# finsberg/fenicsx-beat

Hardware: AMD Instinct MI355X
Metric: node_updates_per_sec (higher is better)
Workload: dtype f64

## Files before the change

### fenicsx-beat_amd/csrc/beat_pde.hip

```cpp
#include "beat_pde_internal.h"

#include <algorithm>
#include <cmath>
#include <cstdlib>
#include <cstring>
#include <vector>

const int beat_pde_detail::kOffsets[45] = {0, 0, 0,  1, 0, 0,  -1, 0, 0,  0, 1, 0,  0, -1, 0,  0, 0, 1,  0, 0, -1,
                          1, 1, 0,  -1, -1, 0,  0, 1, 1,  0, -1, -1,  1, 0, 1,  -1, 0, -1,
                          1, 1, 1,  -1, -1, -1};

namespace {
using namespace beat_pde_detail;

template <int TX_, int TY_>
struct Tile {
  static constexpr int TX = TX_, TY = TY_;
  static constexpr int PITCH = TX + 2;
  static constexpr int SLOT = (TY + 2) * PITCH;
  static constexpr int NLOAD = (SLOT + BEAT_BLOCK - 1) / BEAT_BLOCK;
  static constexpr int ROWS_PER_THREAD = TY / (BEAT_BLOCK / TX);
  static_assert(TX * TY == 1024 && ROWS_PER_THREAD == 4, "tile must hold 1024 nodes");
};
constexpr int TARGET_BLOCKS = 1024;
// ... 243 lines not shown
  }
}

__device__ __forceinline__ void beat_pcg_roll(double* st) {
  st[BETA] = st[RZN] / st[RZ];
  st[RZ] = st[RZN];
  st[RR] = st[RRN];
  st[ITERS] += 1.0;
  const double tr = st[RTOL] * st[RTOL] * st[BB];
  if (st[RR] <= st[TOL2]) {
    st[STOP] = 1.0;
    st[REASON] = st[RR] <= tr ? 2.0 : 3.0;
  } else if (st[ITERS] >= st[MAXIT]) {
    st[STOP] = 1.0;
    st[REASON] = -3.0;
  }
}
__device__ __forceinline__ void beat_pcg_begin(double* st, double rtol, double atol, double max_it) {
  const double bb = st[BB], rr = st[RR];
  const double tr = rtol * rtol * bb, ta = atol * atol;
  const double tol2 = tr > ta ? tr : ta;
  st[TOL2] = tol2;
  st[ITERS] = 0.0;
  st[NUPD] = 0.0;
  st[RTOL] = rtol;
  st[ATOL] = atol;
  st[MAXIT] = max_it;
  st[BETA] = 0.0;
  st[RR0] = rr;
  const bool done = rr <= tol2;
  st[STOP] = done ? 1.0 : 0.0;
  st[REASON] = done ? (rr <= tr ? 2.0 : 3.0) : 0.0;
}
__global__ __launch_bounds__(BEAT_BLOCK) void reduce_partials_kernel(const double* __restrict__ partials, int count, int nsum, double* out,
                                                                     const double* st, double* counter, int then, double* roll_st,
                                                                     double rtol, double atol, double max_it) {
  __shared__ double red[4];
  if (st != nullptr && st[STOP] != 0.0) return;
  if (counter != nullptr && threadIdx.x == 0) counter[0] += 1.0;
  for (int k = 0; k < nsum; ++k) {
    double s = 0.0;
    for (int i = threadIdx.x; i < count; i += BEAT_BLOCK) s += partials[(int64_t)k * BEAT_MAX_PARTIALS + i];
    s = beat_block_sum(s, red);
    if (threadIdx.x == 0) out[k] = s;
  }
  if (then != 0 && threadIdx.x == 0) {
    if (then == 1) beat_pcg_roll(roll_st);
    else beat_pcg_begin(roll_st, rtol, atol, max_it);
  }
}

__global__ void pcg_begin_kernel(double* st, double rtol, double atol, double max_it) { beat_pcg_begin(st, rtol, atol, max_it); }

__global__ void pcg_next_kernel(double* st) {
  if (st[STOP] != 0.0) return;
  beat_pcg_roll(st);
}

template <bool VAR>
__global__ __launch_bounds__(BEAT_BLOCK) void cg_update_kernel(Geom g, const double* __restrict__ st,
                                                               double* __restrict__ x,
                                                               double* __restrict__ r,
                                                               const double* __restrict__ p,
                                                               const double* __restrict__ q,
                                                               const double* __restrict__ dinv,
                                                               double dinv_i, double* __restrict__ partials) {
  __shared__ double red[4];
  if (st[STOP] != 0.0) return;
  const double alpha = st[RZ] / st[PQ];
  const int lane = threadIdx.x & 63, wave = threadIdx.x >> 6;
  const int nrows = g.ny * g.nz;
  double s_rz = 0.0, s_rr = 0.0;
  for (int row = blockIdx.x * 4 + wave; row < nrows; row += gridDim.x * 4) {
    const int iz = row / g.ny, iy = row - iz * g.ny;
    const int tyz = 3 * axis_type(iy, g.ny, 1, 1) + 9 * axis_type(iz, g.nz, g.z_lo_phys, g.z_hi_phys);
    const int64_t base = (int64_t)row * g.nx;
    for (int ix = lane; ix < g.nx; ix += 64) {
      const int type = axis_type(ix, g.nx, 1, 1) + tyz;
      const int64_t i = base + ix;
      const double di = VAR ? dinv[i] : (type == 13) ? dinv_i : dinv[type];
      const double pi = p[i], qi = q[i];
      const double xi = fma(alpha, pi, x[i]);
// ... 184 lines not shown
  g.ny = (int)n[1];
  g.nz = (int)n[2];
  g.plane = n[0] * n[1];
  g.z_lo_phys = z_lo_phys ? 1 : 0;
  g.z_hi_phys = z_hi_phys ? 1 : 0;
  int tile_tx = g.nx >= 256 ? 256 : g.nx >= 128 ? 128 : 64;
  if (const char* e = std::getenv("BEAT_TILE_TX")) {
    const int v = std::atoi(e);
    if (v == 64 || v == 128 || v == 256) tile_tx = v;
  }
  g.tile_tx = tile_tx;
  const int TX = tile_tx, TY = 1024 / tile_tx;
  g.tiles_x = (g.nx + TX - 1) / TX;
  g.tiles_y = (g.ny + TY - 1) / TY;
  const int tiles = g.tiles_x * g.tiles_y;
  int nchunks = std::max(1, (TARGET_BLOCKS + tiles - 1) / tiles);
  nchunks = std::min(nchunks, g.nz);
  g.zc = (g.nz + nchunks - 1) / nchunks;
  g.nchunks = (g.nz + g.zc - 1) / g.zc;
  const int64_t total = (int64_t)tiles * g.nchunks;
  if (total > BEAT_MAX_PARTIALS) {
    g.nchunks = std::max(1, (int)(BEAT_MAX_PARTIALS / tiles));
    g.zc = (g.nz + g.nchunks - 1) / g.nchunks;
    g.nchunks = (g.nz + g.zc - 1) / g.zc;
  }
  BEAT_REQUIRE((int64_t)tiles * g.nchunks <= BEAT_MAX_PARTIALS, "xy plane too large: %d tiles", tiles);
  g.total = tiles * g.nchunks;
  g.z_lo = 0;
  g.z_hi = g.nz;
  g.part_off = 0;
  p->n = n[0] * n[1] * n[2];
  const int64_t rows = (int64_t)g.ny * g.nz;
  p->vec_grid = (unsigned)std::min<int64_t>(2048, std::max<int64_t>(1, (rows + 3) / 4));
  std::memcpy(p->h_mass, host_mass_tab, sizeof(p->h_mass));
  std::memcpy(p->h_stiff, host_stiff_tab, sizeof(p->h_stiff));
  BEAT_HIP_CHECK(hipSetDevice(ctx->device));
  BEAT_HIP_CHECK(hipMalloc(&p->d_tabs, sizeof(double) * (4 * 27 * TABW + 32)));
  BEAT_HIP_CHECK(hipMalloc(&p->d_st, sizeof(double) * BEAT_ST_DOUBLES));
  BEAT_HIP_CHECK(hipMalloc(&p->d_alphas, sizeof(double) * PRING_MAX));
  BEAT_HIP_CHECK(hipMemsetAsync(p->d_st, 0, sizeof(double) * BEAT_ST_DOUBLES, ctx->stream));
  const int rc = upload_tables(p);
  if (rc) return rc;
  *out = p;
  return BEAT_OK;
}


extern "C" int beat_pde_set_ghost_types(beat_pde* pde, int ghost_lo_type, int ghost_hi_type) {
  BEAT_REQUIRE(pde != nullptr, "null pde");
  BEAT_REQUIRE(ghost_lo_type >= 0 && ghost_lo_type <= 2 && ghost_hi_type >= 0 && ghost_hi_type <= 2, "node types are 0, 1 or 2");
  pde->ghost_lo_tz = ghost_lo_type;
  pde->ghost_hi_tz = ghost_hi_type;
  return BEAT_OK;
}

extern "C" int beat_pde_destroy(beat_pde* pde) {
  if (pde == nullptr) return BEAT_OK;
  if (pde->open.on && pde->ctx != nullptr) (void)hipStreamSynchronize(pde->ctx->stream);
  (void)hipFree(pde->d_tabs);
  (void)hipFree(pde->d_st);
  (void)hipFree(pde->d_alphas);
  (void)hipFree(pde->d_batch_st);
  (void)hipFree(pde->d_hist_alloc);
  if (pde->h_st) (void)hipHostFree(pde->h_st);
  if (pde->ev_st) (void)hipEventDestroy(pde->ev_st);
  (void)hipFree(pde->v_A);
// ... 65 lines not shown
}

template <int MODE>
static void launch_stencil(const beat_pde* pde, const StencilArgs& a, const Geom* range = nullptr) {
  const Geom& g = range ? *range : pde->g;
  if (g.total <= 0) return;
  const dim3 grid(stencil_grid(g)), block(BEAT_BLOCK);
  hipStream_t s = pde->ctx->stream;
  switch (g.tile_tx) {
    case 256: BEAT_KERNEL((stencil_kernel<MODE, Tile<256, 4>>), grid, block, 0, s, g, a); break;
    case 128: BEAT_KERNEL((stencil_kernel<MODE, Tile<128, 8>>), grid, block, 0, s, g, a); break;
    default: BEAT_KERNEL((stencil_kernel<MODE, Tile<64, 16>>), grid, block, 0, s, g, a); break;
  }
}

extern "C" int beat_pde_apply(beat_pde* pde, int which, const double* dev_x, double* dev_y) {
  BEAT_REQUIRE(pde != nullptr && dev_x && dev_y, "null argument");
  BEAT_REQUIRE(which >= 0 && which < 4, "which must be 0..3");
  BEAT_REQUIRE(which >= 2 || pde->have_dt, "beat_pde_set_timestep has not been called");
  BEAT_REQUIRE(dev_x != dev_y, "in-place apply is not supported");
  if (pde->var) return beat_var_apply(pde, which, dev_x, dev_y);
  const double* host_tab = which == 0 ? pde->h_A : which == 1 ? pde->h_B : which == 2 ? pde->h_mass : pde->h_stiff;
  StencilArgs a{};
  a.x = dev_x;
  a.y = dev_y;
  a.tab = pde->d_tab(which);
  a.ci = interior(host_tab);
  launch_stencil<MODE_APPLY>(pde, a);
  BEAT_LAUNCH_CHECK();
  return BEAT_OK;
}

int beat_pde_launch_reduce(beat_pde* pde, int count, int nsum, double* out, const double* st, double* counter, int then, double* roll_st,
                           double rtol, double atol, int max_it) {
  static const bool fuse = [] {
    const char* e = std::getenv("BEAT_PCG_FUSE");
    return !(e && e[0] == '0');
  }();
  BEAT_KERNEL(reduce_partials_kernel, dim3(1), dim3(BEAT_BLOCK), 0, pde->ctx->stream, (const double*)pde->ctx->d_partials, count, nsum, out, st,
              counter, fuse ? then : 0, roll_st, rtol, atol, (double)max_it);
  BEAT_LAUNCH_CHECK();
  if (then != 0 && !fuse) {
    if (then == 1) BEAT_KERNEL(pcg_next_kernel, dim3(1), dim3(1), 0, pde->ctx->stream, roll_st);
    else BEAT_KERNEL(pcg_begin_kernel, dim3(1), dim3(1), 0, pde->ctx->stream, roll_st, rtol, atol, (double)max_it);
    BEAT_LAUNCH_CHECK();
  }
  return BEAT_OK;
}

extern "C" int beat_pde_rhs(beat_pde* pde, const double* dev_v_prev, const double* const* host_dev_stim_w,
                            const double* host_stim_amp, int n_stim, double* dev_x, double* dev_r,
                            double* dev_p, double* dev_red) {
  BEAT_REQUIRE(pde != nullptr && dev_v_prev && dev_x && dev_r && dev_p && dev_red, "null argument");
  BEAT_REQUIRE(pde->have_dt, "beat_pde_set_timestep has not been called");
  BEAT_REQUIRE(n_stim >= 0 && n_stim <= BEAT_MAX_STIM, "at most %d stimuli", BEAT_MAX_STIM);
  BEAT_REQUIRE(dev_r != dev_v_prev && dev_p != dev_v_prev && dev_r != dev_p, "r, p must be distinct work fields");
  BEAT_REQUIRE(!pde->guess_pending, "the previous solve's deferred update has not been applied");
  beat_guess_skip(pde);
  if (pde->var)
    return beat_var_rhs(pde, dev_v_prev, host_dev_stim_w, host_stim_amp, n_stim, dev_x, dev_r, dev_p, dev_red);
  StencilArgs a{};
  a.x = dev_v_prev;
  a.y = dev_r;
  a.y2 = dev_p;
  a.y3 = (dev_x == dev_v_prev) ? nullptr : dev_x;
  a.tab = pde->d_tab(2);
  a.tab2 = pde->d_tab(3);
  a.dinv = pde->d_dinv();
  a.ci = interior(pde->h_mass);
  a.ci2 = interior(pde->h_stiff);
  a.dinv_i = pde->h_dinv[13];
  a.cm = pde->C_m;
  a.omt_dt = (1.0 - pde->theta) * pde->dt;
  a.dt = pde->dt;
  a.nstim = 0;
  for (int k = 0; k < n_stim; ++k) {
// ... 401 lines not shown
  }
  beat_guess_advance(pde);
  return due;
}

extern "C" int beat_pde_solve(beat_pde* pde, const double* dev_v_prev,
                              const double* const* host_dev_stim_w, const double* host_stim_amp,
                              int n_stim, double* dev_x, double* dev_work, double rtol, double atol,
                              int max_it, beat_ksp_info* info) {
  return beat_pde_solve_ex(pde, dev_v_prev, host_dev_stim_w, host_stim_amp, n_stim, dev_x, dev_work, rtol, atol, max_it,
                           0, info, nullptr);
}

bool beat_solve_lazy_available(const beat_pde* pde) {
  return pde != nullptr && pde->g.z_lo_phys && pde->g.z_hi_phys && !beat_small_available(pde) && pde->pc_ncoef == 1 &&
         (beat_rr_available(pde) || pde->var);
}

static int solve_enqueue_iterations(beat_pde* pde, int count) {
  beat_pde::OpenSolve& o = pde->open;
  const int64_t fld = beat_pde_field_stride(pde);
  double* r = o.work + pde->g.plane;
  double* q = r + fld;
  double* ring = q + 2 * fld;
  double* st = pde->d_st;
  const int PR = pde->ring;
  int rc;
  for (int it = 0; it < count; ++it) {
    const int i = o.launched + it, slot = i % PR;
    double* p_cur = ring + (int64_t)slot * fld;
    const double* p_old = ring + (int64_t)((i + PR - 1) % PR) * fld;
    if (o.kind == 0) {
      double* rbuf[2] = {r, q};
      if ((rc = beat_rr_pdot(pde, st, rbuf[i & 1], p_old, p_cur))) return rc;
      if ((rc = beat_rr_rupd(pde, st, rbuf[i & 1], rbuf[(i + 1) & 1], p_cur, slot))) return rc;
      if (slot == PR - 1) {
        if ((rc = beat_pde_x_flush_terms(pde, st, o.x, ring, fld, i + 1 - PR, 1, beat_guess_terms(pde, i + 1 - PR)))) return rc;
      }
    } else {
      double* p_next = ring + (int64_t)((i + 1) % PR) * fld;
      if (o.pdot) {
        if ((rc = beat_vtl_pdot(pde, st, r, p_old, p_cur, q, i == 0))) return rc;
      } else if ((rc = beat_pde_spmv_dot(pde, p_cur, q, st))) {
        return rc;
      }
      if ((rc = o.pdot ? beat_var_update_r(pde, st, r, q, slot, true) : beat_pde_cg_update_r(pde, st, r, q, slot))) return rc;
      if (slot == PR - 1) {
        if ((rc = beat_pde_x_flush_terms(pde, st, o.x, ring, fld, i + 1 - PR, 1, beat_guess_terms(pde, i + 1 - PR)))) return rc;
      }
      if (!o.pdot && (rc = beat_pde_cg_next_oop(pde, st, r, p_cur, p_next))) return rc;
    }
  }
  o.launched += count;
  return BEAT_OK;
}

int beat_solve_begin(beat_pde* pde, const double* dev_v_prev, const double* const* host_dev_stim_w, const double* host_stim_amp, int n_stim,
                     double* dev_x, double* dev_work, double rtol, double atol, int max_it) {
  BEAT_REQUIRE(pde != nullptr && dev_work != nullptr && dev_v_prev && dev_x, "null argument");
  BEAT_REQUIRE(beat_solve_lazy_available(pde), "this operator's solves are not of the kind that can be left open");
  BEAT_REQUIRE(!pde->open.on, "the previous solve has not been finished (beat_pde_solve_end)");
  BEAT_REQUIRE(max_it >= 0, "max_it must be >= 0");
  BEAT_REQUIRE(pde->have_dt, "beat_pde_set_timestep has not been called");
  BEAT_REQUIRE(n_stim >= 0 && n_stim <= BEAT_MAX_STIM, "at most %d stimuli", BEAT_MAX_STIM);
  BEAT_REQUIRE(!pde->guess_pending, "the previous solve's deferred update has not been applied");
  beat_ctx* ctx = pde->ctx;
  if (pde->h_st == nullptr) {
// ... 213 lines not shown
```

### fenicsx-beat_amd/csrc/beat_pde_internal.h

```cpp
#pragma once
#include "beat_common.h"

#include <algorithm>
#include <cstdlib>
#include <vector>

namespace beat_pde_detail {

enum St { BB = 0, RZ, RR, PQ, RZN, RRN, TOL2, BETA, STOP, ITERS, REASON, RTOL, ATOL, MAXIT, NUPD, RR0, ALPHA };
constexpr int BEAT_ST_DOUBLES = 32;
constexpr int PRING = 6;
constexpr int PRING_MAX = 12;
constexpr int TABW = 16;

extern const int kOffsets[45];

struct Geom {
  int nx, ny, nz;
  int64_t plane;
  int tiles_x, tiles_y, nchunks, zc, total;
  int z_lo_phys, z_hi_phys;
  int tile_tx;
  int z_lo, z_hi;
  int part_off;
};

enum { MODE_APPLY = 0, MODE_SPMV_DOT = 1, MODE_RHS = 2, MODE_PC = 3 };

}

struct beat_pde {
  beat_ctx* ctx = nullptr;
  beat_pde_detail::Geom g{};
  int64_t n = 0;
  double h_mass[27 * 15], h_stiff[27 * 15];
  double h_A[27 * 15], h_B[27 * 15], h_dinv[27];
  bool have_dt = false;
  double C_m = 1.0, theta = 0.5, dt = 0.0;
  double* d_tabs = nullptr;
  double* d_st = nullptr;
  int last_iters = -1;
  int z_last_iters = -1;
  unsigned vec_grid = 1;
  double* d_alphas = nullptr;
  struct OpenSolve {
    bool on = false;
    int kind = 0;
    bool pdot = false;
    const double* v_prev = nullptr;
    double* x = nullptr;
    double* work = nullptr;
    double rtol = 0.0, atol = 0.0;
    int max_it = 0, launched = 0;
    void* comm = nullptr;
    bool rr = false, merged = false, vpdot = false;
    int limit = 0;
  } open;
  struct FuseBegin {
    bool on = false, done = false;
    double rtol = 0.0, atol = 0.0;
    int max_it = 0;
  } fuse_begin;
  double* h_st = nullptr;
  hipEvent_t ev_st = nullptr;
  beat_ksp_info last_info{};
  bool applied_behind = false;
  beat_pde_detail::GuessTerms applied_terms{};
  int last_rc = 0;
  int ring = beat_pde_detail::PRING;
  int last_base = 0;
  double* d_batch_st = nullptr;
  int ghost_lo_tz = 1, ghost_hi_tz = 1;
  int single_reduction = -1;
  int guess_order = 0;
  int auto_cur = 3;
  int auto_next = 3;
  int auto_e_order = 0;
  double auto_score[4] = {0.0, 0.0, 0.0, 0.0};
  int auto_seen[4] = {0, 0, 0, 0};
  int auto_since_probe = 0, auto_probe_up = 1;
  double* d_hist[3] = {nullptr, nullptr, nullptr};
  double* d_guess = nullptr;
  double* d_hist_alloc = nullptr;
  int hist_fields = 0;
  int hist_n = 0;
  beat_pde_detail::GuessTerms guess{};
  bool guess_pending = false;
  beat_pde_detail::GuessTerms guess_final{};
  int rhs_part_blocks = 0;
  void* vrr = nullptr;
  int vrr_part_blocks = 0;
  void* vtl = nullptr;
  bool small_enabled = true;
  int pc_ncoef = 1;
  double pc_coef[8] = {1.0};
  bool var = false;
  const double* v_mass = nullptr;
  const double* v_stiff = nullptr;
  double* v_A = nullptr;
  double* v_dinv = nullptr;
  double* v_B = nullptr;
  double* v_gc0 = nullptr;
  bool v_gc0_valid = false;
  bool v_pdot_dist = false;
  int64_t v_ld = 0;
  int* v_seg = nullptr;
  std::vector<int> h_seg;
  unsigned long long* v_segmask = nullptr;
  int* v_seg_tiled = nullptr;
  unsigned long long* v_segmask_tiled = nullptr;
  const double* d_tab(int which) const { return d_tabs + (size_t)which * 27 * beat_pde_detail::TABW; }
  const double* d_dinv() const { return d_tabs + (size_t)4 * 27 * beat_pde_detail::TABW; }
  const double* dinv_arg() const { return var ? v_dinv : d_dinv(); }
};

inline int beat_pde_first_chunk(const beat_pde* pde) {
  static const int extra = [] {
    const char* e = std::getenv("BEAT_CHUNK_EXTRA");
    return e ? std::max(0, std::atoi(e)) : 1;
  }();
  return pde->last_iters >= 0 ? std::max(1, pde->last_iters + extra) : 8;
}

int beat_pde_launch_reduce(beat_pde* pde, int count, int nsum, double* out, const double* st, double* counter = nullptr, int then = 0,
                           double* roll_st = nullptr, double rtol = 0.0, double atol = 0.0, int max_it = 0);

int beat_var_form_A(beat_pde* pde);
int beat_var_apply(beat_pde* pde, int which, const double* dev_x, double* dev_y);
int beat_var_rhs(beat_pde* pde, const double* dev_v_prev, const double* const* host_dev_stim_w,
                 const double* host_stim_amp, int n_stim, double* dev_x, double* dev_r, double* dev_p, double* dev_red,
                 const double* dev_e = nullptr,
                 int part = -1);
int beat_var_spmv_dot(beat_pde* pde, const double* dev_p, double* dev_q, double* dev_st);
int beat_var_spmv_dot_part(beat_pde* pde, const double* dev_p, double* dev_q, double* dev_st, int part);
int beat_var_update_r(beat_pde* pde, double* dev_st, double* dev_r, const double* dev_q, int slot, bool roll = false);
int beat_var_pupdate_oop(beat_pde* pde, double* dev_st, const double* dev_r, const double* dev_p_cur, double* dev_p_next);
int beat_var_flush(beat_pde* pde, const double* dev_st, double* dev_x, const double* dev_ring0, int64_t field_stride,
                   int ring_base, int only_if_full, const beat_pde_detail::GuessTerms& gt);

void beat_guess_begin(beat_pde* pde);
void beat_guess_skip(beat_pde* pde);
beat_pde_detail::GuessTerms beat_guess_terms(const beat_pde* pde, int ring_base);
bool beat_guess_end(beat_pde* pde, int nupd, bool deferred);
int beat_pde_x_flush_terms(beat_pde* pde, const double* dev_st, double* dev_x, const double* dev_ring0, int64_t field_stride,
                           int ring_base, int only_if_full, const beat_pde_detail::GuessTerms& gt);

void beat_guess_advance(beat_pde* pde);
void beat_guess_observe(beat_pde* pde, int iterations);
int beat_guess_policy(beat_pde* pde);

int beat_vrr_setup(beat_pde* pde, const std::vector<unsigned long long>& host_tissue_flags);
void beat_vrr_destroy(beat_pde* pde);
bool beat_vrr_available(const beat_pde* pde);
int beat_vrr_spmv_dot(beat_pde* pde, const double* dev_p, double* dev_q, double* dev_st, int part);

int beat_vtl_setup(beat_pde* pde, const std::vector<unsigned long long>& host_tissue_flags);
void beat_vtl_destroy(beat_pde* pde);
bool beat_vtl_available(const beat_pde* pde);
int beat_vtl_spmv_dot(beat_pde* pde, const double* dev_p, double* dev_q, double* dev_st);
bool beat_vtl_parts_available(const beat_pde* pde);
bool beat_vtl_pdot_dist_available(const beat_pde* pde);
int beat_vtl_pdot_part(beat_pde* pde, double* dev_st, const double* dev_r, const double* dev_p_old, double* dev_p_new, double* dev_q,
                       int first, int part);
int beat_vtl_spmv_dot_part(beat_pde* pde, const double* dev_p, double* dev_q, double* dev_st, int part);
bool beat_vtl_pdot_available(const beat_pde* pde);
bool beat_vtl_rhs_available(const beat_pde* pde);
bool beat_vtl_rhs_wanted(const beat_pde* pde);
int beat_vtl_rhs(beat_pde* pde, const double* dev_v_prev, const double* const* host_dev_stim_w, const double* host_stim_amp, int n_stim,
                 double* dev_x, double* dev_r, double* dev_p, double* dev_t, double* dev_red, const double* dev_e);
int beat_vtl_pdot(beat_pde* pde, double* dev_st, const double* dev_r, const double* dev_p_old, double* dev_p_new, double* dev_q, int first);

bool beat_solve_lazy_available(const beat_pde* pde);
struct beat_comm;
int beat_dist_solve_begin(beat_pde* pde, beat_comm* comm, const double* dev_v_prev, const double* const* host_dev_stim_w,
                          const double* host_stim_amp, int n_stim, double* dev_x, double* dev_work, double rtol, double atol, int max_it);
int beat_dist_solve_end(beat_pde* pde, int defer_flush, beat_ksp_info* info, int* host_pending, bool* needed_more);
int beat_solve_begin(beat_pde* pde, const double* dev_v_prev, const double* const* host_dev_stim_w, const double* host_stim_amp, int n_stim,
                     double* dev_x, double* dev_work, double rtol, double atol, int max_it);
int beat_solve_end(beat_pde* pde, int defer_flush, beat_ksp_info* info, int* host_pending, bool* needed_more);

bool beat_small_available(const beat_pde* pde);
int beat_small_launch(beat_pde* pde, const double* dev_v_prev, const double* const* host_dev_stim_w,
                      const double* host_stim_amp, int n_stim, double* dev_x, double rtol, double atol, int max_it,
                      double* dev_st);
int beat_small_solve(beat_pde* pde, const double* dev_v_prev, const double* const* host_dev_stim_w,
                     const double* host_stim_amp, int n_stim, double* dev_x, double rtol, double atol, int max_it,
                     beat_ksp_info* info);

bool beat_rr_available(const beat_pde* pde);
int beat_rr_rhs(beat_pde* pde, const double* dev_v_prev, const double* const* host_dev_stim_w, const double* host_stim_amp,
                int n_stim, double* dev_x, double* dev_r, double* dev_st, int part = -1);
int beat_rr_pdot(beat_pde* pde, double* dev_st, const double* dev_r, const double* dev_p_old, double* dev_p_new);
int beat_rr_pdot_part(beat_pde* pde, double* dev_st, const double* dev_r, const double* dev_p_old, double* dev_p_new,
                      int part);
int beat_rr_rupd(beat_pde* pde, double* dev_st, const double* dev_r, double* dev_r_new, const double* dev_p, int slot,
                 bool roll = true);
int beat_rr_next(beat_pde* pde, double* dev_st);
int beat_rr_udot_part(beat_pde* pde, double* dev_st, const double* dev_r, int part);
int beat_rr_merged_next(beat_pde* pde, double* dev_st, int slot);
int beat_rr_prupd(beat_pde* pde, double* dev_st, const double* dev_r, const double* dev_p_old, double* dev_p_new,
                  double* dev_r_new);
```

### fenicsx-beat_amd/csrc/beat_pde_rr.hip

```cpp
#include "beat_pde_internal.h"

#include <algorithm>
#include <cmath>
#include <cstddef>
#include <cstdlib>

namespace {
using namespace beat_pde_detail;

constexpr int SEG = 62;

struct Coef {
  double c[15];
};

struct RGeom {
  int nx, ny, nz;
  int64_t plane;
  int ry;
  int nsegx, nrb, nchunks, zc;
  int total_waves, total_blocks;
  int z_lo_phys, z_hi_phys;
  int z_lo, z_hi;
  int part_off;
// ... 75 lines not shown
  const int hi = __builtin_amdgcn_update_dpp(__builtin_amdgcn_readlane(__double2hiint(h), src_lane), __double2hiint(v), 0x138, 0xf, 0xf, false);
  return __hiloint2double(hi, lo);
}
__device__ __forceinline__ double from_right_h(double v, double h, int src_lane) {
  const int lo = __builtin_amdgcn_update_dpp(__builtin_amdgcn_readlane(__double2loint(h), src_lane), __double2loint(v), 0x130, 0xf, 0xf, false);
  const int hi = __builtin_amdgcn_update_dpp(__builtin_amdgcn_readlane(__double2hiint(h), src_lane), __double2hiint(v), 0x130, 0xf, 0xf, false);
  return __hiloint2double(hi, lo);
}
#ifndef BEAT_RR_ALIGN_RHS
#define BEAT_RR_ALIGN_RHS 0
#endif
constexpr bool rr_aligned_mode(int mode) {
  return BEAT_RR_ALIGN == 1 && BEAT_RR_BUF != 0 && (mode == 0 || mode == 1 || mode == 3 || mode == 4 || (mode == 2 && BEAT_RR_ALIGN_RHS == 1));
}

__device__ __forceinline__ int axis_type3(int i, int n, int lo_phys, int hi_phys) {
  if (n == 1 && lo_phys && hi_phys) return 1;
  if (i == 0 && lo_phys) return 0;
  if (i == n - 1 && hi_phys) return 2;
  return 1;
}

__device__ __forceinline__ int xcd_block(int b, int total) {
  const int per = (total + 7) >> 3;
  return (b & 7) * per + (b >> 3);
}

#ifndef BEAT_RR_WAVES_RHS
#define BEAT_RR_WAVES_RHS 3
#endif
#ifndef BEAT_RR_WAVES_IT
#define BEAT_RR_WAVES_IT 1
#endif
template <int MODE, int RY, int PD, bool GUESS = false>
__global__ __launch_bounds__(BEAT_BLOCK, (GUESS && RY == 2 && PD == 1) ? BEAT_RR_WAVES_RHS : ((MODE == RR_PDOT || MODE == RR_RUPD) && PD == 1 ? BEAT_RR_WAVES_IT : 1)) void rr_kernel(RGeom g, RArgs a, const double* __restrict__ X,
                                                        const double* __restrict__ X2, double* __restrict__ Y,
                                                        double* __restrict__ Y2) {
  constexpr int NR = RY + 2;
  constexpr int NE = GUESS ? NR : 1;
  constexpr bool FORM = MODE == RR_PDOT || MODE == RR_UDOT || MODE == RR_PRUPD;
  constexpr bool OLD = MODE == RR_PDOT || MODE == RR_PRUPD;
  constexpr bool RAW = MODE == RR_UDOT || MODE == RR_PRUPD;
  constexpr int NW = RAW ? RY : 1;
  constexpr bool BUF = BEAT_RR_BUF == 1 || (BEAT_RR_BUF == 2 && (MODE != RR_RHS || BEAT_RR_ALIGN_RHS == 1));
  constexpr bool ALIGNED = rr_aligned_mode(MODE);
  static_assert(!ALIGNED || BUF, "aligned segments come with the raw-buffer loads");
  constexpr int SEGW = ALIGNED ? 64 : SEG;
  static_assert(!GUESS || MODE == RR_RHS, "the initial guess enters the right-hand side only");
  __shared__ double red[4];
  __shared__ double s_dinv[32];
  __shared__ double s_tab[27 * TABW];
  __shared__ double s_tab2[MODE == RR_RHS ? 27 * TABW : 1];
  __shared__ double s_taba[GUESS ? 27 * TABW : 1];
  if (MODE != RR_RHS) {
    if (a.st[STOP] != 0.0) return;
  }
  for (int i = threadIdx.x; i < 27 * TABW; i += BEAT_BLOCK) {
    s_tab[i] = a.tab[i];
    if (MODE == RR_RHS) s_tab2[i] = a.tab2[i];
    if (GUESS) s_taba[i] = a.taba[i];
  }
  if (threadIdx.x < 27) s_dinv[threadIdx.x] = a.dinv[threadIdx.x];
  __syncthreads();
  const int lane = threadIdx.x & 63;
  const int blk = xcd_block(blockIdx.x, g.total_blocks);
  const int w = blk * 4 + (threadIdx.x >> 6);
  int seg = w % g.nsegx;
  int rb = (w / g.nsegx) % g.nrb;
  int chunk = w / (g.nsegx * g.nrb);
  bool wave_ok = blk < g.total_blocks && w < g.total_waves;
  if (g.nrg > 0) {
    seg = blk % g.nsegx;
    rb = ((blk / g.nsegx) % g.nrg) * 4 + (int)(threadIdx.x >> 6);
    chunk = blk / (g.nsegx * g.nrg);
    wave_ok = blk < g.total_blocks && rb < g.nrb;
  }
  const int gx = seg * SEGW + (ALIGNED ? 0 : -1) + lane;
  const int y0 = rb * RY - 1;
  const int zb = g.z_lo + chunk * g.zc;
  const int ze = wave_ok ? min(zb + g.zc, g.z_hi) : zb;
  const bool x_in = wave_ok && gx >= 0 && gx < g.nx;
  const bool x_out = x_in && (ALIGNED || (lane >= 1 && lane <= SEG));
  const int tx = axis_type3(gx, g.nx, 1, 1);
  bool row_in[NR];
  int txy[NR];
  int off[NR];
  const int cx = min(max(gx, 0), g.nx - 1);
#pragma unroll
  for (int r = 0; r < NR; ++r) {
// ... 53 lines not shown
  for (int zz = zb - 2 - PD; zz < ze; zz += PD) {
#pragma unroll
  for (int u = 0; u < PD; ++u) {
    const int z = zz + u;
    if (z < ze) {
    const int k = z + 1;
    if (k >= zb - 1 && k <= ze) {
      [[maybe_unused]] const bool zok = (k >= 0 || !g.z_lo_phys) && (k < g.nz || !g.z_hi_phys);
      const int tz9 = 9 * (k < 0 ? g.ghost_lo_tz : k >= g.nz ? g.ghost_hi_tz : axis_type3(k, g.nz, g.z_lo_phys, g.z_hi_phys));
      const bool own_plane = (k >= zb && k < ze) || (k == -1 && zb == 0 && !g.z_lo_phys) ||
                             (k == g.nz && ze == g.nz && !g.z_hi_phys);
#pragma unroll
      for (int r = 0; r < NR; ++r) {
        double c = ra[u][r];
        if (RAW && r >= 1 && r <= RY) Rwp[RAW ? r - 1 : 0] = c;
        if (FORM) {
          const int type = txy[r] + tz9;
          const double di = s_dinv[type];
          c = have_old ? fma(beta, rb2[u][r], di * ra[u][r]) : di * ra[u][r];
        }
        if constexpr (!BUF) c = (zok && row_in[r]) ? c : 0.0;
        Cp[r] = c;
        if (GUESS) {
          constexpr int q = GUESS ? 1 : 0;
          if constexpr (BUF)
            Ep[r * q] = c + re1[u][r * q];
          else
            Ep[r * q] = (zok && row_in[r]) ? c + re1[u][r * q] : 0.0;
        }
        if (OLD) {
          if (own_plane && r >= 1 && r <= RY && x_out && row_in[r])
            rr_store(&Y[(int64_t)k * g.plane + (int64_t)(y0 + r) * g.nx + gx], c);
        }
      }
      if constexpr (ALIGNED) {
        double hc = rha[u];
        if (FORM) {
          const double di = s_dinv[htxy + tz9];
          hc = have_old ? fma(beta, rhb[u], di * rha[u]) : di * rha[u];
        }
        Hp = hc;
        if (GUESS) HEp = hc + rhb[u];
      }
    }
    double rv[RY];
    if (MODE == RR_RUPD) {
#pragma unroll
      for (int j = 0; j < RY; ++j) rv[j] = rvn[u][j];
      if (z + PD >= zb && z + PD < ze) {
        const double* __restrict__ br = X2 + (int64_t)(z + PD) * g.plane;
#pragma unroll
        for (int j = 0; j < RY; ++j) rvn[u][j] = BUF ? rr_buf_load(br, pbytes, (unsigned)off[j + 1]) : br[off[j + 1]];
      }
    }
    {
      const int kf = k + PD;
      if (kf >= zb - 1 && kf <= ze) {
        const int cz = min(max(kf, -1), g.nz);
        const double* __restrict__ bx = X + (int64_t)cz * g.plane;
        const double* __restrict__ bx2 = (OLD && have_old) ? X2 + (int64_t)cz * g.plane : bx;
        if constexpr (BUF) {
          const unsigned pb = ((kf >= 0 || !g.z_lo_phys) && (kf < g.nz || !g.z_hi_phys)) ? pbytes : 0u;
#pragma unroll
          for (int r = 0; r < NR; ++r) {
            ra[u][r] = rr_buf_load(bx, pb, (unsigned)off[r]);
            if (OLD) rb2[u][r] = rr_buf_load(bx2, pb, (unsigned)off[r]);
// ... 113 lines not shown
            ev[8] = eL0[rm];
            ev[9] = Ep[rp];
            ev[10] = Em[rm];
            ev[11] = eRp[re_];
            ev[12] = eLm[re_];
            ev[13] = eRp[rp];
            ev[14] = eLm[rm];
            double se = 0.0;
            if (type != 13) {
#pragma unroll
              for (int k = 0; k < 15; ++k) se = fma(s_taba[type * TABW + k], ev[k], se);
            } else {
#pragma unroll
              for (int k = 0; k < 15; ++k) se = fma(az.cia.c[k], ev[k], se);
            }
            rr -= se;
          }
          const double zz = di * rr;
          rr_store(&Y[gi], rr);
          if (Y2 != nullptr) Y2[gi] = v[0];
          acc0 = fma(b, b, acc0);
          acc1 = fma(rr, zz, acc1);
          acc2 = fma(rr, rr, acc2);
        } else {
          double di = s_dinv[13];
          if (type != 13) {
            s = 0.0;
#pragma unroll
            for (int k = 0; k < 15; ++k) s = fma(s_tab[type * TABW + k], v[k], s);
            di = s_dinv[type];
          }
          if (MODE == RR_PDOT) {
            acc0 = fma(v[0], s, acc0);
          } else if (MODE == RR_UDOT) {
            const double ri = Rw0[RAW ? j : 0];
            acc0 = fma(v[0], s, acc0);
            acc1 = fma(ri, v[0], acc1);
            acc2 = fma(ri, ri, acc2);
          } else if (MODE == RR_PRUPD) {
            rr_store(&Y2[gi], fma(-alpha, s, Rw0[RAW ? j : 0]));
          } else {
            const double ri = fma(-alpha, s, rv[j]);
            rr_store(&Y[gi], ri);
            acc0 = fma(ri * di, ri, acc0);
            acc1 = fma(ri, ri, acc1);
          }
        }
      }
    }
    }
#pragma unroll
    for (int r = 0; r < NR; ++r) {
      Cm[r] = C0[r];
      C0[r] = Cp[r];
    }
    if constexpr (ALIGNED) {
      Hm = H0;
      H0 = Hp;
      if (GUESS) {
        HEm = HE0;
        HE0 = HEp;
      }
    }
    if (GUESS) {
#pragma unroll
      for (int r = 0; r < NE; ++r) {
        Em[r] = E0[r];
        E0[r] = Ep[r];
      }
    }
    if (RAW) {
#pragma unroll
      for (int j = 0; j < NW; ++j) Rw0[j] = Rwp[j];
    }
    }
  }
  }

  if (MODE == RR_PDOT) {
    const double s0 = beat_block_sum(acc0, red);
    if (threadIdx.x == 0) a.partials[g.part_off + blockIdx.x] = s0;
  } else if (MODE == RR_RUPD) {
    const double s0 = beat_block_sum(acc0, red);
    const double s1 = beat_block_sum(acc1, red);
    if (threadIdx.x == 0) {
      a.partials[g.part_off + blockIdx.x] = s0;
      a.partials[BEAT_MAX_PARTIALS + g.part_off + blockIdx.x] = s1;
    }
  } else if (MODE == RR_PRUPD) {
  } else {
    const double s0 = beat_block_sum(acc0, red);
    const double s1 = beat_block_sum(acc1, red);
    const double s2 = beat_block_sum(acc2, red);
    if (threadIdx.x == 0) {
      a.partials[g.part_off + blockIdx.x] = s0;
      a.partials[BEAT_MAX_PARTIALS + g.part_off + blockIdx.x] = s1;
      a.partials[2 * BEAT_MAX_PARTIALS + g.part_off + blockIdx.x] = s2;
    }
  }
}

__global__ void rr_next_kernel(double* st) {
  if (st[STOP] != 0.0) return;
  st[BETA] = st[RZN] / st[RZ];
  st[RZ] = st[RZN];
  st[RR] = st[RRN];
  st[ITERS] += 1.0;
  const double tr = st[RTOL] * st[RTOL] * st[BB];
  if (st[RR] <= st[TOL2]) {
    st[STOP] = 1.0;
    st[REASON] = st[RR] <= tr ? 2.0 : 3.0;
  } else if (st[ITERS] >= st[MAXIT]) {
// ... 80 lines not shown
  g.nsegx = (f.nx + segw - 1) / segw;
  g.nrb = (f.ny + RY - 1) / RY;
  const int nzr = std::max(0, z_hi - z_lo);
  g.nrg = (mode >= 0 && ((rr_by_rows_mask() >> mode) & 1)) ? (g.nrb + 3) / 4 : 0;
  const int64_t per_layer = g.nrg > 0 ? (int64_t)g.nsegx * g.nrg : ((int64_t)g.nsegx * g.nrb + 3) / 4;
  const int target = rr_target_blocks(nodes);
  int nchunks = (int)std::max<int64_t>(1, (target + per_layer - 1) / per_layer);
  nchunks = std::max(1, std::min(nchunks, nzr));
  g.zc = std::max(1, (nzr + nchunks - 1) / nchunks);
  g.nchunks = (nzr + g.zc - 1) / g.zc;
  while ((int64_t)g.nsegx * g.nrb * g.nchunks > (int64_t)2 * BEAT_MAX_PARTIALS && g.nchunks > 1) {
    g.zc *= 2;
    g.nchunks = (nzr + g.zc - 1) / g.zc;
  }
  g.total_waves = g.nsegx * g.nrb * g.nchunks;
  g.total_blocks = (g.total_waves + 3) / 4;
  if (g.nrg > 0) {
    g.total_blocks = g.nsegx * g.nrg * g.nchunks;
    g.total_waves = g.total_blocks * 4;
  }
  return g;
}

RGeom make_geom(const beat_pde* pde) { return make_geom(pde, 0, pde->g.nz, 0); }

inline int grid_blocks(const RGeom& g) { return ((g.total_blocks + 7) / 8) * 8; }

Coef interior_row(const double* tab) {
  Coef c;
  for (int k = 0; k < 15; ++k) c.c[k] = tab[13 * 15 + k];
  return c;
}

template <int MODE, bool GUESS = false>
void launch_rr(const beat_pde* pde, const RGeom& g, const RArgs& a) {
  if (g.total_blocks <= 0) return;
  const dim3 grid((unsigned)grid_blocks(g)), block(BEAT_BLOCK);
  hipStream_t s = pde->ctx->stream;
#define BEAT_RR_LAUNCH(RYV, PDV) \
  BEAT_KERNEL((rr_kernel<MODE, RYV, PDV, GUESS>), grid, block, 0, s, g, a, a.x, GUESS ? a.e : a.x2, a.y, a.y2)
  const int pd = rr_prefetch();
  if (g.ry == 2) {
    if (pd == 2) BEAT_RR_LAUNCH(2, 2); else if (pd == 3) BEAT_RR_LAUNCH(2, 3); else BEAT_RR_LAUNCH(2, 1);
  } else {
    if (pd == 2) BEAT_RR_LAUNCH(4, 2); else if (pd == 3) BEAT_RR_LAUNCH(4, 3); else BEAT_RR_LAUNCH(4, 1);
  }
#undef BEAT_RR_LAUNCH
}
}

bool beat_rr_available(const beat_pde* pde) {
  if (pde->var || pde->pc_ncoef != 1) return false;
  if (const char* e = std::getenv("BEAT_RR")) {
    if (e[0] == '0') return false;
  }
  const RGeom g = make_geom(pde);
  const RGeom gb = make_geom(pde, 0, 1, 0);
  return (int64_t)grid_blocks(g) + 2 * grid_blocks(gb) <= BEAT_MAX_PARTIALS;
}

int beat_rr_rhs(beat_pde* pde, const double* dev_v_prev, const double* const* host_dev_stim_w, const double* host_stim_amp,
                int n_stim, double* dev_x, double* dev_r, double* dev_st, int part) {
  const GuessTerms& gt = pde->guess;
  const bool guess = gt.d != nullptr && gt.use_e;
  static const int guess_rows = [] {
    const char* e = std::getenv("BEAT_RR_GUESS_RY");
    const int v = e ? std::atoi(e) : 2;
    return v == 4 ? 4 : 2;
  }();
  const int rows = guess ? guess_rows : 0;
  RArgs a{};
  a.x = dev_v_prev;
  a.y = dev_r;
// ... 26 lines not shown
  auto launch = [&](const RGeom& g) {
    if (guess)
      launch_rr<RR_RHS, true>(pde, g, a);
    else
      launch_rr<RR_RHS>(pde, g, a);
    return g.total_blocks > 0 ? grid_blocks(g) : 0;
  };
  const Geom& f = pde->g;
  if (part < 0) {
    const int nb = launch(make_geom(pde, 0, f.nz, 0, rows, RR_RHS));
    BEAT_LAUNCH_CHECK();
    if (pde->fuse_begin.on) {
      pde->fuse_begin.done = true;
      return beat_pde_launch_reduce(pde, nb, 3, dev_st, nullptr, nullptr, 2, dev_st, pde->fuse_begin.rtol, pde->fuse_begin.atol,
                                    pde->fuse_begin.max_it);
    }
    return beat_pde_launch_reduce(pde, nb, 3, dev_st, nullptr);
  }
  const int lo = f.z_lo_phys ? 0 : 1, hi = f.nz - (f.z_hi_phys ? 0 : 1);
  const RGeom gi = make_geom(pde, lo, std::max(lo, hi), 0, rows, RR_RHS);
  if (part == 0) {
    launch(gi);
    BEAT_LAUNCH_CHECK();
    return BEAT_OK;
  }
  int off = gi.total_blocks > 0 ? grid_blocks(gi) : 0;
  if (!f.z_lo_phys) off += launch(make_geom(pde, 0, 1, off, rows, RR_RHS));
  if (!f.z_hi_phys && (f.nz > 1 || f.z_lo_phys)) off += launch(make_geom(pde, f.nz - 1, f.nz, off, rows, RR_RHS));
  BEAT_LAUNCH_CHECK();
  BEAT_REQUIRE(off <= BEAT_MAX_PARTIALS, "too many block partials");
  return beat_pde_launch_reduce(pde, off, 3, dev_st, nullptr);
}

int beat_rr_pdot_part(beat_pde* pde, double* dev_st, const double* dev_r, const double* dev_p_old, double* dev_p_new,
                      int part) {
  const Geom& f = pde->g;
  RArgs a{};
  a.x = dev_r;
  a.x2 = dev_p_old;
  a.y = dev_p_new;
  a.tab = pde->d_tab(0);
  a.dinv = pde->d_dinv();
  a.ci = interior_row(pde->h_A);
  a.dinv_i = pde->h_dinv[13];
  a.partials = pde->ctx->d_partials;
  a.st = dev_st;
  const int lo = f.z_lo_phys ? 0 : 1, hi = f.nz - (f.z_hi_phys ? 0 : 1);
  const RGeom gi = make_geom(pde, lo, std::max(lo, hi), 0, 0, RR_PDOT);
  if (part == 0) {
    launch_rr<RR_PDOT>(pde, gi, a);
    BEAT_LAUNCH_CHECK();
    return BEAT_OK;
  }
  int off = gi.total_blocks > 0 ? grid_blocks(gi) : 0;
  if (!f.z_lo_phys) {
    const RGeom gb = make_geom(pde, 0, 1, off, 0, RR_PDOT);
    launch_rr<RR_PDOT>(pde, gb, a);
    off += grid_blocks(gb);
  }
  if (!f.z_hi_phys && (f.nz > 1 || f.z_lo_phys)) {
    const RGeom gb = make_geom(pde, f.nz - 1, f.nz, off, 0, RR_PDOT);
    launch_rr<RR_PDOT>(pde, gb, a);
    off += grid_blocks(gb);
  }
  BEAT_LAUNCH_CHECK();
  BEAT_REQUIRE(off <= BEAT_MAX_PARTIALS, "too many block partials");
  return beat_pde_launch_reduce(pde, off, 1, dev_st + PQ, dev_st);
}

int beat_rr_pdot(beat_pde* pde, double* dev_st, const double* dev_r, const double* dev_p_old, double* dev_p_new) {
  if (int rc = beat_rr_pdot_part(pde, dev_st, dev_r, dev_p_old, dev_p_new, 0)) return rc;
  return beat_rr_pdot_part(pde, dev_st, dev_r, dev_p_old, dev_p_new, 1);
}

int beat_rr_rupd(beat_pde* pde, double* dev_st, const double* dev_r, double* dev_r_new, const double* dev_p, int slot,
                 bool roll) {
  const RGeom g = make_geom(pde, 0, pde->g.nz, 0, 0, RR_RUPD);
  RArgs a{};
  a.x = dev_p;
  a.x2 = dev_r;
  a.y = dev_r_new;
  a.tab = pde->d_tab(0);
  a.dinv = pde->d_dinv();
  a.ci = interior_row(pde->h_A);
  a.dinv_i = pde->h_dinv[13];
  a.partials = pde->ctx->d_partials;
  a.st = dev_st;
  a.alphas = pde->d_alphas;
  a.slot = slot;
  launch_rr<RR_RUPD>(pde, g, a);
  BEAT_LAUNCH_CHECK();
  return beat_pde_launch_reduce(pde, grid_blocks(g), 2, dev_st + RZN, dev_st, dev_st + NUPD, roll ? 1 : 0, dev_st);
}

int beat_rr_udot_part(beat_pde* pde, double* dev_st, const double* dev_r, int part) {
  static_assert(RZN == PQ + 1 && RRN == PQ + 2, "the three sums travel as one all-reduce of dev_st[PQ..RRN]");
  const Geom& f = pde->g;
  RArgs a{};
  a.x = dev_r;
  a.x2 = dev_r;
  a.tab = pde->d_tab(0);
  a.dinv = pde->d_dinv();
  a.ci = interior_row(pde->h_A);
  a.dinv_i = pde->h_dinv[13];
  a.partials = pde->ctx->d_partials;
// ... 55 lines not shown
```

Measured before the change: 10.79 billion.

## Predict CG convergence in the p-dot pass to skip the final residual update

The p-dot kernel now also accumulates r·q and q·q next to p·q, and the reduction kernel gains a predict mode. Using these three sums it computes the next residual norm by recurrence, with a floating-point error bound derived from the reduction depth. When that prediction safely decides convergence, it writes alpha and stops the solve, so the separate residual-update pass and its reduction are skipped on the last iteration. The cost is extra shared-memory traffic and two more dot products in every p-dot pass. It only runs when both z boundaries are physical and is on by default.

```diff
diff --git a/fenicsx-beat_amd/csrc/beat_pde.hip b/fenicsx-beat_amd/csrc/beat_pde.hip
--- a/fenicsx-beat_amd/csrc/beat_pde.hip
+++ b/fenicsx-beat_amd/csrc/beat_pde.hip
@@ -299,9 +299,30 @@
   st[STOP] = done ? 1.0 : 0.0;
   st[REASON] = done ? (rr <= tr ? 2.0 : 3.0) : 0.0;
 }
+__device__ __forceinline__ void beat_pcg_predict(double* st, double* alpha_slot, double c) {
+  st[PQ] = st[PQS];
+  const double alpha = st[RZ] / st[PQ];
+  const double rr = st[RR], rq = st[RQ], qq = st[QQ];
+  const double rho = fma(alpha, fma(alpha, qq, -2.0 * rq), rr);
+  const double m = sqrt(rr) + fabs(alpha) * sqrt(qq);
+  const double e = c * m * m;
+  const double tr = st[RTOL] * st[RTOL] * st[BB];
+  if (!(rho + e <= st[TOL2]) || !(e <= 0x1p-20 * rho)) return;
+  double reason;
+  if (rho + e <= tr) reason = 2.0;
+  else if (rho - e > tr) reason = 3.0;
+  else return;
+  *alpha_slot = alpha;
+  st[RR] = rho > 0.0 ? rho : 0.0;
+  st[ITERS] += 1.0;
+  st[NUPD] += 1.0;
+  st[REASON] = reason;
+  st[STOP] = 1.0;
+}
 __global__ __launch_bounds__(BEAT_BLOCK) void reduce_partials_kernel(const double* __restrict__ partials, int count, int nsum, double* out,
                                                                      const double* st, double* counter, int then, double* roll_st,
-                                                                     double rtol, double atol, double max_it) {
+                                                                     double rtol, double atol, double max_it, double* alpha_slot,
+                                                                     double bound_c) {
   __shared__ double red[4];
   if (st != nullptr && st[STOP] != 0.0) return;
   if (counter != nullptr && threadIdx.x == 0) counter[0] += 1.0;
@@ -313,8 +334,14 @@
   }
   if (then != 0 && threadIdx.x == 0) {
     if (then == 1) beat_pcg_roll(roll_st);
+    else if (then == 3) beat_pcg_predict(roll_st, alpha_slot, bound_c);
     else beat_pcg_begin(roll_st, rtol, atol, max_it);
   }
+}
+
+__global__ void pcg_predict_kernel(double* st, double* alpha_slot, double c) {
+  if (st[STOP] != 0.0) return;
+  beat_pcg_predict(st, alpha_slot, c);
 }
 
 __global__ void pcg_begin_kernel(double* st, double rtol, double atol, double max_it) { beat_pcg_begin(st, rtol, atol, max_it); }
@@ -565,6 +592,7 @@
   p->n = n[0] * n[1] * n[2];
   const int64_t rows = (int64_t)g.ny * g.nz;
   p->vec_grid = (unsigned)std::min<int64_t>(2048, std::max<int64_t>(1, (rows + 3) / 4));
+  if (const char* e = std::getenv("BEAT_PCG_PREDICT_STOP")) p->predict_stop = e[0] != '0';
   std::memcpy(p->h_mass, host_mass_tab, sizeof(p->h_mass));
   std::memcpy(p->h_stiff, host_stiff_tab, sizeof(p->h_stiff));
   BEAT_HIP_CHECK(hipSetDevice(ctx->device));
@@ -696,16 +724,17 @@
 }
 
 int beat_pde_launch_reduce(beat_pde* pde, int count, int nsum, double* out, const double* st, double* counter, int then, double* roll_st,
-                           double rtol, double atol, int max_it) {
+                           double rtol, double atol, int max_it, double* alpha_slot, double bound_c) {
   static const bool fuse = [] {
     const char* e = std::getenv("BEAT_PCG_FUSE");
     return !(e && e[0] == '0');
   }();
   BEAT_KERNEL(reduce_partials_kernel, dim3(1), dim3(BEAT_BLOCK), 0, pde->ctx->stream, (const double*)pde->ctx->d_partials, count, nsum, out, st,
-              counter, fuse ? then : 0, roll_st, rtol, atol, (double)max_it);
+              counter, fuse ? then : 0, roll_st, rtol, atol, (double)max_it, alpha_slot, bound_c);
   BEAT_LAUNCH_CHECK();
   if (then != 0 && !fuse) {
     if (then == 1) BEAT_KERNEL(pcg_next_kernel, dim3(1), dim3(1), 0, pde->ctx->stream, roll_st);
+    else if (then == 3) BEAT_KERNEL(pcg_predict_kernel, dim3(1), dim3(1), 0, pde->ctx->stream, roll_st, alpha_slot, bound_c);
     else BEAT_KERNEL(pcg_begin_kernel, dim3(1), dim3(1), 0, pde->ctx->stream, roll_st, rtol, atol, (double)max_it);
     BEAT_LAUNCH_CHECK();
   }
@@ -1173,7 +1202,7 @@
     const double* p_old = ring + (int64_t)((i + PR - 1) % PR) * fld;
     if (o.kind == 0) {
       double* rbuf[2] = {r, q};
-      if ((rc = beat_rr_pdot(pde, st, rbuf[i & 1], p_old, p_cur))) return rc;
+      if ((rc = beat_rr_pdot(pde, st, rbuf[i & 1], p_old, p_cur, slot))) return rc;
       if ((rc = beat_rr_rupd(pde, st, rbuf[i & 1], rbuf[(i + 1) & 1], p_cur, slot))) return rc;
       if (slot == PR - 1) {
         if ((rc = beat_pde_x_flush_terms(pde, st, o.x, ring, fld, i + 1 - PR, 1, beat_guess_terms(pde, i + 1 - PR)))) return rc;
diff --git a/fenicsx-beat_amd/csrc/beat_pde_internal.h b/fenicsx-beat_amd/csrc/beat_pde_internal.h
--- a/fenicsx-beat_amd/csrc/beat_pde_internal.h
+++ b/fenicsx-beat_amd/csrc/beat_pde_internal.h
@@ -7,7 +7,7 @@
 
 namespace beat_pde_detail {
 
-enum St { BB = 0, RZ, RR, PQ, RZN, RRN, TOL2, BETA, STOP, ITERS, REASON, RTOL, ATOL, MAXIT, NUPD, RR0, ALPHA };
+enum St { BB = 0, RZ, RR, PQ, RZN, RRN, TOL2, BETA, STOP, ITERS, REASON, RTOL, ATOL, MAXIT, NUPD, RR0, ALPHA, PQS, RQ, QQ };
 constexpr int BEAT_ST_DOUBLES = 32;
 constexpr int PRING = 6;
 constexpr int PRING_MAX = 12;
@@ -69,6 +69,8 @@
   int last_rc = 0;
   int ring = beat_pde_detail::PRING;
   int last_base = 0;
+  bool predict_stop = true;
+  double predict_c = 0.0;
   double* d_batch_st = nullptr;
   int ghost_lo_tz = 1, ghost_hi_tz = 1;
   int single_reduction = -1;
@@ -123,7 +125,8 @@
 }
 
 int beat_pde_launch_reduce(beat_pde* pde, int count, int nsum, double* out, const double* st, double* counter = nullptr, int then = 0,
-                           double* roll_st = nullptr, double rtol = 0.0, double atol = 0.0, int max_it = 0);
+                           double* roll_st = nullptr, double rtol = 0.0, double atol = 0.0, int max_it = 0, double* alpha_slot = nullptr,
+                           double bound_c = 0.0);
 
 int beat_var_form_A(beat_pde* pde);
 int beat_var_apply(beat_pde* pde, int which, const double* dev_x, double* dev_y);
@@ -190,9 +193,10 @@
 bool beat_rr_available(const beat_pde* pde);
 int beat_rr_rhs(beat_pde* pde, const double* dev_v_prev, const double* const* host_dev_stim_w, const double* host_stim_amp,
                 int n_stim, double* dev_x, double* dev_r, double* dev_st, int part = -1);
-int beat_rr_pdot(beat_pde* pde, double* dev_st, const double* dev_r, const double* dev_p_old, double* dev_p_new);
+int beat_rr_pdot(beat_pde* pde, double* dev_st, const double* dev_r, const double* dev_p_old, double* dev_p_new, int slot = -1);
 int beat_rr_pdot_part(beat_pde* pde, double* dev_st, const double* dev_r, const double* dev_p_old, double* dev_p_new,
-                      int part);
+                      int part, int slot = -1);
+double beat_rr_predict_bound(const beat_pde* pde);
 int beat_rr_rupd(beat_pde* pde, double* dev_st, const double* dev_r, double* dev_r_new, const double* dev_p, int slot,
                  bool roll = true);
 int beat_rr_next(beat_pde* pde, double* dev_st);
diff --git a/fenicsx-beat_amd/csrc/beat_pde_rr.hip b/fenicsx-beat_amd/csrc/beat_pde_rr.hip
--- a/fenicsx-beat_amd/csrc/beat_pde_rr.hip
+++ b/fenicsx-beat_amd/csrc/beat_pde_rr.hip
@@ -131,7 +131,7 @@
 #ifndef BEAT_RR_WAVES_IT
 #define BEAT_RR_WAVES_IT 1
 #endif
-template <int MODE, int RY, int PD, bool GUESS = false>
+template <int MODE, int RY, int PD, bool GUESS = false, bool PRED = false>
 __global__ __launch_bounds__(BEAT_BLOCK, (GUESS && RY == 2 && PD == 1) ? BEAT_RR_WAVES_RHS : ((MODE == RR_PDOT || MODE == RR_RUPD) && PD == 1 ? BEAT_RR_WAVES_IT : 1)) void rr_kernel(RGeom g, RArgs a, const double* __restrict__ X,
                                                         const double* __restrict__ X2, double* __restrict__ Y,
                                                         double* __restrict__ Y2) {
@@ -146,14 +146,18 @@
   static_assert(!ALIGNED || BUF, "aligned segments come with the raw-buffer loads");
   constexpr int SEGW = ALIGNED ? 64 : SEG;
   static_assert(!GUESS || MODE == RR_RHS, "the initial guess enters the right-hand side only");
+  static_assert(!PRED || MODE == RR_PDOT, "the predicted-stop sums come with PDOT only");
   __shared__ double red[4];
   __shared__ double s_dinv[32];
   __shared__ double s_tab[27 * TABW];
   __shared__ double s_tab2[MODE == RR_RHS ? 27 * TABW : 1];
   __shared__ double s_taba[GUESS ? 27 * TABW : 1];
+  __shared__ double s_rc[PRED ? 4 * 2 * RY * 64 : 1];
+  __shared__ double s_acc[PRED ? 4 * 2 * 64 : 1];
   if (MODE != RR_RHS) {
     if (a.st[STOP] != 0.0) return;
   }
+  if (PRED) s_acc[(threadIdx.x >> 6) * 128 + (threadIdx.x & 63)] = s_acc[(threadIdx.x >> 6) * 128 + 64 + (threadIdx.x & 63)] = 0.0;
   for (int i = threadIdx.x; i < 27 * TABW; i += BEAT_BLOCK) {
     s_tab[i] = a.tab[i];
     if (MODE == RR_RHS) s_tab2[i] = a.tab2[i];
@@ -273,6 +277,7 @@
           if (own_plane && r >= 1 && r <= RY && x_out && row_in[r])
             rr_store(&Y[(int64_t)k * g.plane + (int64_t)(y0 + r) * g.nx + gx], c);
         }
+        if (PRED && r >= 1 && r <= RY) s_rc[((((threadIdx.x >> 6) * 2 + (k & 1)) * RY) + r - 1) * 64 + lane] = ra[u][r];
       }
       if constexpr (ALIGNED) {
         double hc = rha[u];
@@ -452,6 +457,11 @@
           }
           if (MODE == RR_PDOT) {
             acc0 = fma(v[0], s, acc0);
+            if (PRED) {
+              double* sa = &s_acc[(threadIdx.x >> 6) * 128 + lane];
+              sa[0] = fma(s_rc[((((threadIdx.x >> 6) * 2 + (z & 1)) * RY) + j) * 64 + lane], s, sa[0]);
+              sa[64] = fma(s, s, sa[64]);
+            }
           } else if (MODE == RR_UDOT) {
             const double ri = Rw0[RAW ? j : 0];
             acc0 = fma(v[0], s, acc0);
@@ -497,7 +507,11 @@
   }
   }
 
-  if (MODE == RR_PDOT) {
+  if (PRED) {
+    acc1 = s_acc[(threadIdx.x >> 6) * 128 + (threadIdx.x & 63)];
+    acc2 = s_acc[(threadIdx.x >> 6) * 128 + 64 + (threadIdx.x & 63)];
+  }
+  if (MODE == RR_PDOT && !PRED) {
     const double s0 = beat_block_sum(acc0, red);
     if (threadIdx.x == 0) a.partials[g.part_off + blockIdx.x] = s0;
   } else if (MODE == RR_RUPD) {
@@ -644,13 +658,13 @@
   return c;
 }
 
-template <int MODE, bool GUESS = false>
+template <int MODE, bool GUESS = false, bool PRED = false>
 void launch_rr(const beat_pde* pde, const RGeom& g, const RArgs& a) {
   if (g.total_blocks <= 0) return;
   const dim3 grid((unsigned)grid_blocks(g)), block(BEAT_BLOCK);
   hipStream_t s = pde->ctx->stream;
 #define BEAT_RR_LAUNCH(RYV, PDV) \
-  BEAT_KERNEL((rr_kernel<MODE, RYV, PDV, GUESS>), grid, block, 0, s, g, a, a.x, GUESS ? a.e : a.x2, a.y, a.y2)
+  BEAT_KERNEL((rr_kernel<MODE, RYV, PDV, GUESS, PRED>), grid, block, 0, s, g, a, a.x, GUESS ? a.e : a.x2, a.y, a.y2)
   const int pd = rr_prefetch();
   if (g.ry == 2) {
     if (pd == 2) BEAT_RR_LAUNCH(2, 2); else if (pd == 3) BEAT_RR_LAUNCH(2, 3); else BEAT_RR_LAUNCH(2, 1);
@@ -743,9 +757,26 @@
   return beat_pde_launch_reduce(pde, off, 3, dev_st, nullptr);
 }
 
+double beat_rr_predict_bound(const beat_pde* pde) {
+  const Geom& f = pde->g;
+  int depth = 0;
+  auto chain = [&](const RGeom& g) {
+    const int per_thread = (grid_blocks(g) + BEAT_BLOCK - 1) / BEAT_BLOCK;
+    depth = std::max(depth, g.zc * g.ry + 8 + per_thread + 8);
+  };
+  chain(make_geom(pde, 0, f.nz, 0, 0, RR_RHS));
+  chain(make_geom(pde, 0, f.nz, 0, 2, RR_RHS));
+  chain(make_geom(pde, 0, f.nz, 0, 4, RR_RHS));
+  chain(make_geom(pde, 0, f.nz, 0, 0, RR_PDOT));
+  chain(make_geom(pde, 0, f.nz, 0, 0, RR_RUPD));
+  return 4.0 * (2.0 * depth + 8.0) * std::ldexp(1.0, -53);
+}
+
 int beat_rr_pdot_part(beat_pde* pde, double* dev_st, const double* dev_r, const double* dev_p_old, double* dev_p_new,
-                      int part) {
+                      int part, int slot) {
   const Geom& f = pde->g;
+  const bool pred = slot >= 0 && pde->predict_stop && f.z_lo_phys && f.z_hi_phys;
+  if (pred && pde->predict_c <= 0.0) pde->predict_c = beat_rr_predict_bound(pde);
   RArgs a{};
   a.x = dev_r;
   a.x2 = dev_p_old;
@@ -756,32 +787,43 @@
   a.dinv_i = pde->h_dinv[13];
   a.partials = pde->ctx->d_partials;
   a.st = dev_st;
+  auto launch = [&](const RGeom& g) {
+    if (pred)
+      launch_rr<RR_PDOT, false, true>(pde, g, a);
+    else
+      launch_rr<RR_PDOT>(pde, g, a);
+  };
   const int lo = f.z_lo_phys ? 0 : 1, hi = f.nz - (f.z_hi_phys ? 0 : 1);
   const RGeom gi = make_geom(pde, lo, std::max(lo, hi), 0, 0, RR_PDOT);
   if (part == 0) {
-    launch_rr<RR_PDOT>(pde, gi, a);
+    launch(gi);
     BEAT_LAUNCH_CHECK();
     return BEAT_OK;
   }
   int off = gi.total_blocks > 0 ? grid_blocks(gi) : 0;
   if (!f.z_lo_phys) {
     const RGeom gb = make_geom(pde, 0, 1, off, 0, RR_PDOT);
-    launch_rr<RR_PDOT>(pde, gb, a);
+    launch(gb);
     off += grid_blocks(gb);
   }
   if (!f.z_hi_phys && (f.nz > 1 || f.z_lo_phys)) {
     const RGeom gb = make_geom(pde, f.nz - 1, f.nz, off, 0, RR_PDOT);
-    launch_rr<RR_PDOT>(pde, gb, a);
+    launch(gb);
     off += grid_blocks(gb);
   }
   BEAT_LAUNCH_CHECK();
   BEAT_REQUIRE(off <= BEAT_MAX_PARTIALS, "too many block partials");
+  if (pred) {
+    static_assert(RQ == PQS + 1 && QQ == PQS + 2, "the three sums are reduced into one run of slots");
+    return beat_pde_launch_reduce(pde, off, 3, dev_st + PQS, dev_st, nullptr, 3, dev_st, 0.0, 0.0, 0, pde->d_alphas + slot,
+                                  pde->predict_c);
+  }
   return beat_pde_launch_reduce(pde, off, 1, dev_st + PQ, dev_st);
 }
 
-int beat_rr_pdot(beat_pde* pde, double* dev_st, const double* dev_r, const double* dev_p_old, double* dev_p_new) {
-  if (int rc = beat_rr_pdot_part(pde, dev_st, dev_r, dev_p_old, dev_p_new, 0)) return rc;
-  return beat_rr_pdot_part(pde, dev_st, dev_r, dev_p_old, dev_p_new, 1);
+int beat_rr_pdot(beat_pde* pde, double* dev_st, const double* dev_r, const double* dev_p_old, double* dev_p_new, int slot) {
+  if (int rc = beat_rr_pdot_part(pde, dev_st, dev_r, dev_p_old, dev_p_new, 0, slot)) return rc;
+  return beat_rr_pdot_part(pde, dev_st, dev_r, dev_p_old, dev_p_new, 1, slot);
 }
 
 int beat_rr_rupd(beat_pde* pde, double* dev_st, const double* dev_r, double* dev_r_new, const double* dev_p, int slot,
```

After: 11.30 billion, median of 6. +4.8%, better.
